# xmlyqing00/V-FloodNet

Hardware: AMD Instinct MI355X
Metric: segmented frames/sec at 480p (higher is better)
Workload: dtype f32

## Files before the change

### v-floodnet_amd/_lib.py

```python
import ctypes as C
import os
import re

import torch

_HERE = os.path.dirname(os.path.abspath(__file__))
LIB_PATH = os.environ.get('VFN_LIB_PATH') or os.path.join(_HERE, 'libvfn_hip.so')

_lib = None

c_fp = C.c_void_p

_SCALARS = {'int': C.c_int, 'float': C.c_float, 'double': C.c_double, 'long long': C.c_longlong}
_POINTEES = set(_SCALARS) | {'void', 'char', 'unsigned char', 'short', 'unsigned short', 'unsigned long long'}
_RENAMED = {'in': 'inp'}
_DECLARATOR = re.compile(r'(?:const\s+)?([A-Za-z_][\w ]*?)(?:\s*(\*)\s*|\s+)(\w+)\s*(?:\[([^\]]*)\])?')


def parse_header(text, known_structs=None):
    defines, enums, structs, protos = {}, {}, dict(known_structs or {}), {}

    def fail(why, decl):
        raise RuntimeError(f'vfn_hip.h: {why}: {" ".join(decl.split())[:120]!r}')

# ... 48 lines not shown
        depth += (ch == '{') - (ch == '}')
        if depth < 0:
            fail('unbalanced declaration', text[start:pos + 1])
        if ch == ';' and depth == 0:
            decls.append(text[start:pos])
            start = pos + 1
    if text[start:].strip():
        fail('unbalanced declaration', text[start:])

    for decl in decls:
        m = re.fullmatch(r'\s*enum\s*\{(.*)\}\s*', decl, flags=re.S)
        if m:
            value = -1
            for item in m.group(1).split(','):
                name, _, expr = item.partition('=')
                value = number(expr, decl) if expr.strip() else value + 1
                enums[name.strip()] = value
            continue
        m = re.fullmatch(r'\s*typedef\s+struct\s*(\w*)\s*\{(.*)\}\s*(\w+)\s*', decl, flags=re.S)
        if m:
            if m.group(1) not in ('', m.group(3)):
                fail('struct tag and typedef name differ', decl)
            fields = []
            for member in m.group(2).split(';'):
                if member.strip():
                    first, *more = member.split(',')
                    head = _DECLARATOR.fullmatch(first.strip())
                    if more and (not head or head.group(2)):
                        fail('several declarators after a pointer', member)
                    fields.append(declarator(first, member, False))
                    fields += [declarator(f'{head.group(1)} {item}', member, False) for item in more]
            structs[m.group(3)] = type(m.group(3), (C.Structure,), {'_fields_': fields})
            continue
        m = re.fullmatch(r'\s*int\s+(vfn_\w+)\s*\((.*)\)\s*', decl, flags=re.S)
        if m:
            if m.group(1) in protos:
                fail('declared twice', decl)
            params = m.group(2).strip()
            protos[m.group(1)] = [] if params == 'void' else [declarator(p, decl, True)[1] for p in params.split(',')]
            continue
        fail('declaration not understood', decl)
    return defines, enums, {k: v for k, v in structs.items() if k not in (known_structs or {})}, protos


with open(os.path.join(os.path.dirname(_HERE), 'include', 'vfn_hip.h')) as _f:
    DEFINES, ENUMS, STRUCTS, SIGNATURES = parse_header(_f.read())
ALL_SYMBOLS = sorted(SIGNATURES)
with open(os.path.join(os.path.dirname(_HERE), 'include', 'vfn_winograd6.h')) as _f:
    SIGNATURES_WINOGRAD6 = parse_header(_f.read())[3]
with open(os.path.join(os.path.dirname(_HERE), 'include', 'vfn_image_val.h')) as _f:
    DEFINES_IMAGE_VAL, _, _, SIGNATURES_IMAGE_VAL = parse_header(_f.read())
with open(os.path.join(os.path.dirname(_HERE), 'include', 'vfn_shortcut_fused.h')) as _f:
    SIGNATURES_SHORTCUT_FUSED = parse_header(_f.read(), STRUCTS)[3]
SEG_SCORES_CHUNK, SEG_SCORES_MAX_BLOCKS = DEFINES_IMAGE_VAL['VFN_SEG_SCORES_CHUNK'], DEFINES_IMAGE_VAL['VFN_SEG_SCORES_MAX_BLOCKS']
ABI_VERSION = DEFINES['VFN_ABI_VERSION']
TRAIN_AUG_MAX_T, TRAIN_AUG_MAX_SIDE, TRAIN_AUG_MAX_OUT, TRAIN_AUG_MAX_OBJ = (
    DEFINES['VFN_TRAIN_AUG_MAX_' + _k] for _k in ('T', 'SIDE', 'OUT', 'OBJ'))

ConvDesc = STRUCTS['vfn_conv_desc']
WgradDesc = STRUCTS['vfn_wgrad_desc']
RefreshFilter = STRUCTS['vfn_refresh_filter']
RefreshEpilogue = STRUCTS['vfn_refresh_epilogue']
GatherEntry = STRUCTS['vfn_gather_entry']
StemDesc = STRUCTS['vfn_stem_desc']
BankScanDesc = STRUCTS['vfn_bankscan_desc']
MemReadDesc = STRUCTS['vfn_memread_desc']
BankMatchDesc = STRUCTS['vfn_bankmatch_desc']
BankDesc = STRUCTS['vfn_bank_desc']
TrainAugFrame = STRUCTS['vfn_train_aug_frame']
TrainAugDesc = STRUCTS['vfn_train_aug_desc']

DESC_IDS = {ENUMS['VFN_DESC_' + _k]: _c for _k, _c in (
    ('CONV', ConvDesc), ('STEM', StemDesc), ('BANKSCAN', BankScanDesc), ('MEMREAD', MemReadDesc), ('BANK', BankDesc),
    ('WGRAD', WgradDesc), ('REFRESH_FILTER', RefreshFilter), ('REFRESH_EPILOGUE', RefreshEpilogue), ('GATHER', GatherEntry),
    ('BANKMATCH', BankMatchDesc), ('TRAIN_AUG', TrainAugDesc))}


def lib():
    global _lib
    if _lib is None:
        if not os.path.isfile(LIB_PATH):
            raise RuntimeError(
                f'{LIB_PATH} not found: build the HIP kernels first '
                '(python -c "import __graft_entry__ as g; g.build()" or make -C v-floodnet_amd/csrc)')
        L = C.CDLL(LIB_PATH)

        def declare(name, signatures=SIGNATURES, header='vfn_hip.h'):
            if not hasattr(L, name):
                raise RuntimeError(f'{LIB_PATH} lacks {name}, which include/{header} declares: rebuild it (make -C v-floodnet_amd/csrc)')
            fn = getattr(L, name)
            fn.argtypes, fn.restype = signatures[name], C.c_int
            return fn

        if declare('vfn_abi_version')() != ABI_VERSION:
            raise RuntimeError(f'{LIB_PATH} has ABI version {L.vfn_abi_version()}, this package expects {ABI_VERSION} '
                               '(descriptor layouts differ): rebuild it (make -C v-floodnet_amd/csrc)')
        declare('vfn_sizeof_desc')
        for which, cls in DESC_IDS.items():
            if L.vfn_sizeof_desc(which) != C.sizeof(cls):
                raise RuntimeError(f'{LIB_PATH}: sizeof({cls.__name__}) is {L.vfn_sizeof_desc(which)} in the library, '
                                   f'{C.sizeof(cls)} in this binding: rebuild it (make -C v-floodnet_amd/csrc)')
        for name in SIGNATURES:
            declare(name)
        for name in SIGNATURES_WINOGRAD6:
            declare(name, SIGNATURES_WINOGRAD6, 'vfn_winograd6.h')
        for name in SIGNATURES_IMAGE_VAL:
            declare(name, SIGNATURES_IMAGE_VAL, 'vfn_image_val.h')
        for name in SIGNATURES_SHORTCUT_FUSED:
            declare(name, SIGNATURES_SHORTCUT_FUSED, 'vfn_shortcut_fused.h')
        _lib = L
    return _lib


def check(status, what):
    if status != 0:
        raise RuntimeError(f'HIP kernel launcher {what} failed with status {status}')


def ptr(t):
    if t is None:
        return None
    return C.c_void_p(t.data_ptr())


_raw_stream = getattr(torch._C, '_cuda_getCurrentRawStream', None)


def stream():
    if _raw_stream is not None:
        return C.c_void_p(_raw_stream(torch.cuda.current_device()))
    return C.c_void_p(torch.cuda.current_stream().cuda_stream)


def require_gpu(t, what='tensor'):
    if not t.is_cuda:
        raise RuntimeError(f'{what} must live on the GPU: the V-FloodNet hot path has no CPU fallback')


PROBES = []


def independent_stream(device, beside=(), tries=12, priority=0):
    device = torch.device(device)
    cur = torch.cuda.current_stream(device)
    others = [cur] + [s_ for s_ in beside if s_ is not None]
    big, small = torch.zeros(16 * 1024 * 1024, device=device), torch.zeros(16, device=device)

    def overlaps(cand, ref):
        torch.cuda.synchronize(device)
        ref_end, cand_end = torch.cuda.Event(), torch.cuda.Event()
        with torch.cuda.stream(ref):
            for _ in range(64):
                big.add_(1.0)
            ref_end.record()
        with torch.cuda.stream(cand):
            small.add_(1.0)
            cand_end.record()
        cand_end.synchronize()
        ok = not ref_end.query()
        torch.cuda.synchronize(device)
        return ok

# ... 11 lines not shown
```

### v-floodnet_amd/engine.py

```python
import math
import os

import torch

from . import _lib, ops, weights as W
from ._lib import ptr, stream, check, MemReadDesc, BankScanDesc
from .feature_bank import pick_nsplit, pick_scan_slices, MAX_SPLIT, MAX_SPLIT_SCAN, QT_SCAN, DK, DV

_CFG_EFF = {(128, 128): 1.00, (128, 64): 0.95, (64, 128): 0.95, (64, 64): 0.86, (32, 64): 0.74,
            (64, 32): 0.74, (128, 32): 0.80, (256, 128): 0.97}
_CFG_TILES = None
_TUNED = {}
_TUNED_PATH = __import__('os').path.join(__import__('os').path.dirname(__import__('os').path.abspath(__file__)),
                                         'tuned_gfx950.json')
_TUNED_BF16 = {}
_TUNED_BF16_PATH = _TUNED_PATH.replace('tuned_gfx950.json', 'tuned_gfx950_bf16.json')
_TUNED_BF16X3 = {}
_TUNED_BF16X3_PATH = _TUNED_PATH.replace('tuned_gfx950.json', 'tuned_gfx950_bf16x3.json')
_TABLES = (_TUNED, _TUNED_BF16, _TUNED_BF16X3)
_TABLE_PATHS = (_TUNED_PATH, _TUNED_BF16_PATH, _TUNED_BF16X3_PATH)
_TUNED_WINO6 = {}
_TUNED_WINO6_PATH = _TUNED_PATH.replace('tuned_gfx950.json', 'tuned_gfx950_wino6.json')
_TUNED_SHORTCUT = {}
_TUNED_SHORTCUT_PATH = _TUNED_PATH.replace('tuned_gfx950.json', 'tuned_gfx950_shortcut.json')


def is_wino6_desc(d):
    return d.w_batch_rows > 0 and d.M == 64 * d.w_batch_rows


def table_of(d, mode):
    return _TUNED_WINO6 if mode == 0 and is_wino6_desc(d) else _TABLES[mode]


def _load_tuned():
    import json
    import os
    if os.environ.get('VFN_IGNORE_TUNED') == '1':
        return
    for path, table in zip(_TABLE_PATHS + (_TUNED_WINO6_PATH,), _TABLES + (_TUNED_WINO6,)):
        alt = os.environ.get('VFN_TUNED_DIR')
        if alt and os.path.isfile(os.path.join(alt, os.path.basename(path))):
            path = os.path.join(alt, os.path.basename(path))
        if os.path.isfile(path):
            for k, v in json.load(open(path)).items():
                t = (int(v[0]), int(v[1]), int(v[2]) if len(v) > 2 else 0)
                table[tuple(int(x) for x in k.split(','))] = t + tuple(int(x) for x in v[3:6]) if len(v) >= 6 else t
    path = _TUNED_SHORTCUT_PATH
    alt = os.environ.get('VFN_TUNED_DIR')
    if alt and os.path.isfile(os.path.join(alt, os.path.basename(path))):
        path = os.path.join(alt, os.path.basename(path))
    if os.path.isfile(path):
        for k, v in json.load(open(path)).items():
            _TUNED_SHORTCUT[tuple(int(x) for x in k.split(','))] = (int(v[0]), int(v[1]))


def save_tuned(path=None, mode=0):
    import json
    table = _TUNED_WINO6 if mode == 'wino6' else _TUNED_SHORTCUT if mode == 'shortcut' else _TABLES[mode]
    with open(path or (_TUNED_WINO6_PATH if mode == 'wino6' else _TUNED_SHORTCUT_PATH if mode == 'shortcut' else _TABLE_PATHS[mode]), 'w') as f:
        json.dump({','.join(str(x) for x in k): list(v) for k, v in sorted(table.items())}, f, indent=0)


_load_tuned()


def pad_divide_by(h, w, d=16):
    new_h = h + d - h % d if h % d > 0 else h
    new_w = w + d - w % d if w % d > 0 else w
    lh = int((new_h - h) / 2)
    uh = int(new_h - h) - lh
    lw = int((new_w - w) / 2)
    uw = int(new_w - w) - lw
    return (lw, uw, lh, uh), new_h, new_w


WS_FLOATS = 16 * 1024 * 1024
_WINOGRAD_TRAIN = os.environ.get('VFN_WINOGRAD_TRAIN', '1') == '1'
_BATCH_MEMREAD = os.environ.get('VFN_TRAIN_BATCH_MEMREAD', '1') == '1'
MAX_GROUP = 16
_TRAIN_SLOTS = int(os.environ.get('VFN_TRAIN_SLOTS', 2))
_WINOGRAD = os.environ.get('VFN_WINOGRAD', '1')
_WINOGRAD_F6 = os.environ.get('VFN_WINOGRAD_F6', '1')
_WINO_ROWS32 = os.environ.get('VFN_WINO_ROWS32', '1')
_SHORTCUT_FUSED = os.environ.get('VFN_SHORTCUT_FUSED', '1')
_WINOGRAD_LP = os.environ.get('VFN_WINOGRAD_LP', '1') == '1'
_WINOGRAD_MIN_M = int(os.environ.get('VFN_WINOGRAD_MIN_M', 10000))
_WINO_TABLE = {}
_WINO_TABLE_BF16 = {}
_WINO_PATH = os.path.join(os.path.dirname(os.path.abspath(__file__)), 'wino_gfx950.json')
if os.environ.get('VFN_IGNORE_TUNED') != '1':
    for _path, _tab in ((_WINO_PATH, _WINO_TABLE), (_WINO_PATH.replace('.json', '_bf16.json'), _WINO_TABLE_BF16)):
        if os.path.isfile(_path):
            _tab.update({tuple(int(x) for x in k.split(',')): int(v) for k, v in __import__('json').load(open(_path)).items()})
_INLAUNCH_SPLITK = __import__('os').environ.get('VFN_INLAUNCH_SPLITK', '1') == '1'


def _tiles():
    global _CFG_TILES
    if _CFG_TILES is None:
        _CFG_TILES = ops.conv_cfg_tiles()
    return _CFG_TILES


def apply_choice(desc, choice, ws, counters=None):
    cfg, ks, split_from = choice[:3]
    if ks > 1 and (desc.out_ld % 4 or (desc.res and desc.res_ld % 4)):
        ks, split_from = 1, 0
    if cfg >= ops.PCONV_CFG0 and not ops.pconv_eligible(desc, 0):
        fb = tuple(choice[3:6]) if len(choice) >= 6 else choose_cfg(desc.M, desc.Cout, desc.KH * desc.KW * desc.Cin, 0, use_table=False)
        return apply_choice(desc, fb, ws, counters)
    if cfg >= ops.WINO_GEMM_CFG0:
        ops.set_splitk(desc, 1, None)
        return cfg
    if ops.conv_cfg_kind(cfg) == 2:
        if counters is None or ws is None or ws.numel() < ops.SK_WS_FLOATS:
            ws, counters = ops.streamk_scratch(ws.device if ws is not None else torch.device('cuda', torch.cuda.current_device()))
        ops.set_streamk(desc, ws, counters)
        return cfg
    if ks > 1:
        bm, bn = _tiles()[cfg]
        n_tiles = (desc.Cout + bn - 1) // bn
        rows = desc.M - (split_from // n_tiles) * bm
        if desc.Cout % bn or not _INLAUNCH_SPLITK or ops.conv_cfg_kind(cfg) != 0 or desc.w_packed or desc.in_lp or desc.out_lp:
            counters = None
        ops.set_splitk(desc, ks, ws, split_from, rows, counters)
    else:
        ops.set_splitk(desc, 1, None)
    return cfg


def _scores_buffer(p, fb):
    if os.environ.get('VFN_STORE_SCORES', '1') == '0':
        return None
    per_obj = ((fb._cap + 63) // 64) * ((p.HW + 127) // 128) * 8192
    if fb.obj_n * per_obj * 4 > float(os.environ.get('VFN_SCORES_MAX_GB', 48)) * 2 ** 30:
        return None
    key = (fb.obj_n, per_obj)
# ... 379 lines not shown
    def all_lists(self):
        out = [self.mem]
        for qs in self.qsets:
            out += [qs.pre[1], qs.pre[2], qs.post[0], qs.post[1]]
        for qs in self._qbatch.values():
            out += [qs.pre[qs.nq]]
            if qs._dec_batch is not None:
                out += [qs._dec_batch.post]
        return out

    def batch_set(self, n):
        qs = self._qbatch.get(n)
        if qs is None:
            qs = self._qbatch[n] = QuerySet(self, nq=n)
            qs.build()
        return qs

    def _trunk_buffers(self, N):
        dev = self.eng.device
        f = lambda *s: torch.empty(*s, device=dev, dtype=torch.float32)
        b = {}
        b['r1'] = f(N, self.h2, self.w2, 64)
        b['x4'] = f(N, self.h4, self.w4, 64)
        for name, (h, w, planes) in {'res2': (self.h4, self.w4, 64), 'res3': (self.h8, self.w8, 128),
                                     'res4': (self.h16, self.w16, 256)}.items():
            hin, win = (h * 2, w * 2) if name != 'res2' else (h, w)
            b[name] = dict(t1a=f(N, hin, win, planes), t1=f(N, h, w, planes), t2=f(N, h, w, planes),
                           ds=f(N, h, w, planes * 4), o=[f(N, h, w, planes * 4) for _ in range(2)],
                           out=f(N, h, w, planes * 4))
        return b

    def _lp_args(self, out):
        if not self.eng.any_x3 or out.shape[-1] % 32:
            return ()
        self._lp_state[(out.data_ptr(), tuple(out.shape))] = True
        return (self.lp_twin(out), True)

    def lp_twin(self, t):
        st = t.untyped_storage()
        key = st.data_ptr()
        if key not in self._twins:
            self._twins[key] = torch.empty(st.nbytes() // 4, dtype=torch.float32, device=t.device)
        return torch.as_strided(self._twins[key], t.size(), t.stride(), t.storage_offset())

    def has_lp(self, t, relu):
        return self._lp_state.get((t.data_ptr(), tuple(t.shape))) == bool(relu)

    def _conv(self, lst, layer, x, out, N, H, Wd, res=None, relu_in=False, relu_out=False, name='conv',
              in_ld=None, out_ld=None, res_mod=0, lp_out=None, f32_out=True):
        bf = self.eng.layer_mode(name)
        lp = bf == 2
        if self.eng.mixed:
            f32_out = True
        if ((bf == 0 or (bf == 1 and _WINOGRAD_LP and not self.keep_acts and layer.cin % 64 == 0)) and in_ld is None and
                (_WINOGRAD_TRAIN or not self.keep_acts) and x.shape[-1] == layer.cin and self.eng.use_winograd(layer, N * H * Wd, bf)):
            tile = 6 if (bf == 0 and not self.keep_acts and res_mod % (H * Wd) == 0 and
                         self.eng.winograd_tile(layer, N * H * Wd) == 6) else 4
            return self._conv_winograd(lst, layer, x, out, N, H, Wd, res, relu_in, relu_out, name, out_ld, res_mod, bf, tile)
        d = ops.make_conv_desc(x, layer.w, layer.cout, layer.k, layer.k, layer.stride, layer.pad, out,
                               layer.scale, layer.shift, res, relu_in, relu_out,
                               cin=layer.cin, in_ld=in_ld if in_ld is not None else x.shape[-1],
                               out_ld=out_ld, N=N, H=H, W=Wd)
        d.res_mod = int(res_mod)
        if lp and in_ld is None and layer.cin % 32 == 0 and self.has_lp(x, relu_in):
            d.inp, d.in_lp, d.relu_in = ptr(self.lp_twin(x)), 1, 0
        if lp and lp_out and layer.cout % 32 == 0 and d.out_ld % 32 == 0:
            d.out_lp, d.out_lp_relu = ptr(self.lp_twin(out)), int(lp_out == 'relu')
            self._lp_state[(out.data_ptr(), tuple(out.shape))] = (lp_out == 'relu')
            if not f32_out:
                d.out = None
        else:
            self._lp_state.pop((out.data_ptr(), tuple(out.shape)), None)
        K = layer.k * layer.k * layer.cin
        if bf == 1 and layer.cin % 64:
            bf = 2
        if bf:
            ops.use_packed_weights(d, layer.w_lp(bf))
        choice = choose_cfg(d.M, layer.cout, K, bf)
        if choice[1] > 1 and (d.out_ld % 4 or (res is not None and d.res_ld % 4)):
            choice = (choice[0], 1, 0)
        cfg = apply_choice(d, choice, self._ws_cur, self._cnt_cur)
        lst.append(Launch(ops.conv2d_launch, (d, cfg, bf), f'{name}[{d.M}x{layer.cout}x{K}]', 2.0 * d.M * layer.cout * K))
        return out

    def _conv_winograd(self, lst, layer, x, out, N, H, Wd, res, relu_in, relu_out, name, out_ld, res_mod, bf=0, tile=4):
        comps = 64 if tile == 6 else 36
        rows = ops.winograd6_rows(N, H, Wd) if tile == 6 else ops.winograd_rows(N, H, Wd)
        if tile == 6 and bf == 0 and _WINO_ROWS32 != '0':
            rows32 = (ops.winograd6_tiles(N, H, Wd) + 31) // 32 * 32
            c32 = _TUNED_WINO6.get((64 * rows32, layer.cout, layer.cin))
            if rows32 < rows and (_WINO_ROWS32 == '2' or (c32 is not None and ops.is_wino_gemm32_cfg(c32[0]))):
                rows = rows32
        key = id(self._ws_cur)
        need_v, need_m = comps * rows * layer.cin, comps * rows * layer.cout
        V, Mb = self._wino.get(key, (None, None))
        if V is None or V.numel() < need_v or Mb.numel() < need_m:
            dev = self.eng.device
            V = torch.zeros(max(need_v, V.numel() if V is not None else 0), device=dev)
            Mb = torch.empty(max(need_m, Mb.numel() if Mb is not None else 0), device=dev)
            self._wino[key] = (V, Mb)
        Mb = Mb[:need_m].view(comps * rows, layer.cout)
        if bf == 1:
            V = V.view(torch.bfloat16)[:need_v].view(36 * rows, layer.cin)
            U = layer.w_wino_bf16()
        else:
            V = V[:need_v].view(comps * rows, layer.cin)
            U = layer.w_wino6() if tile == 6 else layer.w_wino()
        lst.append(Launch(ops.winograd_input, (x, V, rows, relu_in, N, H, Wd, layer.cin, x.shape[-1], tile), name + '.wino_in'))
        dg = ops.make_winograd_gemm_desc(V, U, Mb, rows, layer.cin, layer.cout, comps)
        if bf:
            choice = _TABLES[bf].get((dg.M, layer.cout, layer.cin))
            if choice is None or choice[0] < ops.WINO_GEMM_CFG0:
                tc = 5 if rows % 64 == 0 and layer.cout >= 128 and rows >= 1024 else 3
                choice = (ops.wino_gemm_cfg(tc, 512), 1, 0)
        elif tile == 6:
            choice = _TUNED_WINO6.get((dg.M, layer.cout, layer.cin))
            if choice is None or choice[0] not in ops.wino_gemm_cfg_options(rows, layer.cout):
                choice = ((ops.wino_gemm32_cfg(4 if layer.cout >= 128 else 5, 768) if rows % 64 else
                           ops.wino_gemm_cfg(5 if layer.cout >= 128 else 7, 768)), 1, 0)
        else:
            choice = choose_cfg(dg.M, layer.cout, layer.cin, 0)
        cfg = apply_choice(dg, choice, self._ws_cur, self._cnt_cur)
        lst.append(Launch(ops.conv2d_launch, (dg, cfg, bf), f'{name}.wino_gemm[{dg.M}x{layer.cout}x{layer.cin}]', 2.0 * dg.M * layer.cout * layer.cin))
        self._lp_state.pop((out.data_ptr(), tuple(out.shape)), None)
        lst.append(Launch(ops.winograd_output, (Mb, rows, out, N, H, Wd, layer.cout, layer.scale, layer.shift, res,
                                                res.shape[-1] if res is not None else 0, res_mod, relu_out,
                                                out_ld if out_ld is not None else out.shape[-1], tile), name + '.wino_out'))
        return out

    def _trunk(self, lst, enc, bufs, N, prefix, acts=None):
        x = bufs['x4']
        lst.append(Launch(ops.maxpool3x3s2, (bufs['r1'], x), prefix + '.maxpool'))
        H, Wd = self.h4, self.w4
        for lname in ('res2', 'res3', 'res4'):
            blocks = enc[lname]
            lb = bufs[lname]
            for bi, blk in enumerate(blocks):
                s = blk['conv2'].stride
                Ho, Wo = H // s, Wd // s
                t1 = lb['t1a'] if (s == 2) else lb['t1']
                t2, ds_buf = lb['t2'], lb['ds']
                if self.keep_acts:
                    t1, t2 = torch.empty_like(t1), torch.empty_like(lb['t2'])
                    ds_buf = torch.empty_like(lb['ds'])
                nm = f'{prefix}.{lname}.{bi}'
                self._conv(lst, blk['conv1'], x, t1, N, H, Wd, relu_out=True, name=nm + '.conv1', lp_out='plain', f32_out=False)
                self._conv(lst, blk['conv2'], t1, t2, N, H, Wd, relu_out=True, name=nm + '.conv2', lp_out='plain',
                           f32_out=False)
                out = lb['out'] if bi == len(blocks) - 1 else lb['o'][bi % 2]
                if self.keep_acts and bi != len(blocks) - 1:
                    out = torch.empty_like(out)
                if 'down' in blk and self._shortcut_fused(lst, blk, x, t2, out, N, H, Wd, Ho, Wo, nm):
                    idn = None
                elif 'down' in blk:
                    self._conv(lst, blk['down'], x, ds_buf, N, H, Wd, name=nm + '.down')
                    idn = ds_buf
                else:
                    idn = x
                if idn is not None:
                    self._conv(lst, blk['conv3'], t2, out, N, Ho, Wo, res=idn, relu_out=True, name=nm + '.conv3',
                               lp_out='plain')
# ... 709 lines not shown
        m.q = ptr(kv_q)
        m.qv = None
        m.bank_k, m.bank_v, m.bank_len, m.ml, m.o_part = ptr(fb._kbuf), ptr(fb._vbuf), ptr(fb._len_dev), ptr(p.ml), ptr(p.o_part)
        m.cnt = ptr(fb._cnt) if update_bank else None
        m.info, m.out = ptr(fb._ibuf), ptr(out)
        m.stride_k, m.stride_v, m.stride_cnt, m.stride_info = cap * DK, cap * DV, cap, cap * 2
        m.scale, m.thres = scale, 1e-3
        m.ldq, m.ldqv, m.ld_out, m.HW, m.obj_n = DK + DV, DK + DV, out.shape[-1], HW, K
        m.precision = mr_mode
        m.nsplit = pick_nsplit(HW, K, fb.len_upper(), QT_SCAN, MAX_SPLIT)
        if klp is not None:
            m.bank_k_lp, m.bank_v_lp = ptr(klp), ptr(vlp)
        if scores is not None:
            m.scores, m.stride_scores = ptr(scores), scores.shape[1]
        check(L.vfn_memread_apply(_lib.C.byref(m), s), 'vfn_memread_apply')
        check(L.vfn_memread_finish(_lib.C.byref(m), s), 'vfn_memread_finish')

    def capture(self, H0, W0, obj_n, group=0):
        p = self.plan(H0, W0, obj_n)
        if not _GRAPHS or self.eager or p.keep_acts:
            return 0
        before = p.graphs.captures
        torch.cuda.current_stream().synchronize()
        p.graphs.warm(p.mem)
        for qs in p.qsets:
            for n in qs.sizes:
                lst = qs.pre[n]
                p.graphs.warm(lst)
                if 0 < qs.split[n] < len(lst):
                    p.graphs.warm(lst, 0, qs.split[n])
                    p.graphs.warm(lst, qs.split[n], None)
            for L in qs.post:
                p.graphs.warm(L)
        for G in ([group] if group and group > 1 else []):
            qs = p.batch_set(G)
            b = qs.dec_batch()
            if self.refresher._tables is None:
                self._settle()
            p.graphs.warm(qs.pre[G])
            p.graphs.warm(b.post)
        torch.cuda.current_stream().synchronize()
        return p.graphs.captures - before

    def autotune(self, H0, W0, obj_n, iters=3, only_missing=False, shape_filter=None, cfg_filter=None):
        p = self.plan(H0, W0, obj_n)
        seen = {}
        side_sets = list(p.qsets) + ([] if p.keep_acts else list(p._qbatch.values()))
        side_lists = [id(qs.pre[n]) for qs in side_sets for n in qs.sizes]
        for lst in p.all_lists():
            for l in lst:
                l_side = id(lst) in side_lists
                if l.fn is ops.conv2d_launch:
                    d = l.args[0]
                    key = (d.M, d.Cout, d.KH * d.KW * d.Cin, int(l.args[2]), is_wino6_desc(d))
                    if only_missing and key[:3] in table_of(d, key[3]):
                        continue
                    if shape_filter is not None and not shape_filter(key[:3]):
                        continue
                    seen.setdefault(key, []).append((l, l_side))
        for key, launches in seen.items():
            d = launches[0][0].args[0]
            bf = key[3]
            if key[4]:
                best = tune_desc(d, bf, p.ws, p.cnt, iters=iters, cfg_filter=lambda k_, c_: c_ >= ops.WINO_GEMM_CFG0 and (cfg_filter is None or cfg_filter(k_, c_)))
            else:
                best = tune_desc(d, bf, p.ws, p.cnt, iters=iters, cfg_filter=cfg_filter)
            table_of(d, bf)[key[:3]] = best
            for l, in_q in launches:
                l.args = (l.args[0], apply_choice(l.args[0], best, p.ws_q if in_q else p.ws, p.cnt_q if in_q else p.cnt), bf)
        if seen:
            p.graphs.invalidate()
        return dict(_TABLES[self.mode])
```

### v-floodnet_amd/ops.py

```python
import ctypes as C
import os

import torch

from . import _lib
from ._lib import ptr, stream, check, ConvDesc


_cfg_tiles = None


def conv_cfg_tiles():
    global _cfg_tiles
    if _cfg_tiles is None:
        L = _lib.lib()
        out = []
        for c in range(L.vfn_conv_cfg_count()):
            bm, bn = C.c_int(), C.c_int()
            L.vfn_conv_cfg_tile(c, C.byref(bm), C.byref(bn))
            out.append((bm.value, bn.value))
        _cfg_tiles = tuple(out)
    return _cfg_tiles


# ... 208 lines not shown


def pconv_cfg(tile_cfg, wgs=512):
    return PCONV_CFG0 + int(tile_cfg) + 8 * (int(wgs) // 128)


def pconv_eligible(desc, mode=0):
    lim = 0x7fffff00
    return (mode == 0 and desc.KH == 1 and desc.KW == 1 and desc.stride == 1 and desc.pad == 0 and not desc.mask and not desc.in_lp and
            not desc.out_lp and not desc.w_packed and not desc.w_batch_rows and desc.Cin % 32 == 0 and desc.in_ld % 4 == 0 and
            desc.M >= 1 and desc.M == desc.N * desc.H * desc.W and desc.M * desc.in_ld * 4 < lim and desc.M * desc.out_ld * 4 < lim and
            desc.cout_pad * desc.Cin * 4 < lim and
            (not desc.res or (desc.res_mod if desc.res_mod > 0 else desc.M) * desc.res_ld * 4 < lim))


def shortcut_fused_eligible(sc, main, mode=0):
    lim = 0x7fffff00
    for d in (sc, main):
        if (d.KH != 1 or d.KW != 1 or d.pad != 0 or d.mask or d.in_lp or d.out_lp or d.w_packed or d.ksplit > 1 or d.w_batch_rows or d.res or
                d.Cin < 32 or d.Cin % 32 or d.in_ld < d.Cin or d.in_ld % 4 or d.N < 1 or d.H < 1 or d.W < 1 or not d.inp or not d.w):
            return False
    return (mode == 0 and bool(main.out) and main.stride == 1 and sc.stride in (1, 2) and main.M >= 1 and main.M == main.N * main.H * main.W and
            sc.Ho == (sc.H - 1) // sc.stride + 1 and sc.Wo == (sc.W - 1) // sc.stride + 1 and sc.M == sc.N * sc.Ho * sc.Wo and
            sc.M == main.M and sc.Cout == main.Cout and main.Cout >= 1 and main.out_ld >= main.Cout and
            min(sc.cout_pad, main.cout_pad) >= (main.Cout + 63) // 64 * 64 and
            sc.N * sc.H * sc.W * sc.in_ld * 4 < lim and main.M * main.in_ld * 4 < lim and main.M * main.out_ld * 4 < lim and
            main.cout_pad * main.Cin * 4 < lim and sc.cout_pad * sc.Cin * 4 < lim)


def shortcut_fused_cfg_options(sc, main):
    out = []
    for tc in range(4):
        bn = WINO_GEMM_TILES[tc & 3][1]
        if (bn > 64 and main.Cout < 128) or min(sc.cout_pad, main.cout_pad) < (main.Cout + bn - 1) // bn * bn:
            continue
        out += [(tc, w) for w in (256, 512, 768)]
    return out


def shortcut_fused_launch(sc, main, tile_cfg, wgs):
    check(_lib.lib().vfn_conv1x1_shortcut_fused_f32(C.byref(sc), C.byref(main), int(tile_cfg), int(wgs), stream()),
          'vfn_conv1x1_shortcut_fused_f32')


def pconv_cfg_options(cout):
    out = []
    for tc in range(8):
        if WINO_GEMM_TILES[tc & 3][1] > 64 and cout < 128:
            continue
        out += [pconv_cfg(tc, w) for w in (256, 512, 768)]
    return out


def conv2d_launch(desc, cfg, mode=0):
    cfg = int(cfg)
    if cfg >= PCONV_CFG0:
        c = cfg - PCONV_CFG0
        if mode != 0:
            raise RuntimeError('the persistent 1x1 convolution is an f32 kernel')
        check(_lib.lib().vfn_conv1x1_persistent_f32(C.byref(desc), c & 7, (c >> 3) * 128, stream()), 'vfn_conv1x1_persistent_f32')
        return
    if cfg >= WINO_GEMM_CFG0:
        c, rows = cfg - WINO_GEMM_CFG0, desc.w_batch_rows
        if is_wino_gemm32_cfg(cfg):
            c = cfg - WINO_GEMM32_CFG0
            if mode != 0 or rows <= 0:
                raise RuntimeError('the 32-row tiles take an f32 Winograd-domain descriptor (w_batch_rows)')
            check(_lib.lib().vfn_winograd_gemm_f32(desc.inp, desc.w, desc.out, desc.M // rows, rows, desc.Cin, desc.Cout, desc.cout_pad,
                                                   8 + (c & 7), (c >> 3) * 128, stream()), 'vfn_winograd_gemm_f32')
            return
        if mode == 1 and rows > 0:
            check(_lib.lib().vfn_winograd_gemm_bf16(desc.inp, desc.w, desc.out, desc.M // rows, rows, desc.Cin, desc.Cout, desc.cout_pad, c & 7,
                                                    (c >> 3) * 128, stream()), 'vfn_winograd_gemm_bf16')
            return
        if mode != 0 or rows <= 0:
            raise RuntimeError('the persistent GEMM takes an f32 (or plain-bf16) Winograd-domain descriptor (w_batch_rows)')
        check(_lib.lib().vfn_winograd_gemm_f32(desc.inp, desc.w, desc.out, desc.M // rows, rows, desc.Cin, desc.Cout, desc.cout_pad, c & 7,
                                               (c >> 3) * 128, stream()), 'vfn_winograd_gemm_f32')
        return
    name = _CONV_FN[int(mode)]
    check(getattr(_lib.lib(), name)(C.byref(desc), cfg, stream()), name)


def conv_cfg_name(cfg, mode=0, _cache={}):
    cfg = int(cfg)
    if cfg >= WINO_GEMM_CFG0:
        bm, bn, wm, wn, pd, _ = persistent_cfg_info(cfg)
        return f'wino_gemm_kernel<{bm}, {bn}, {wm}, {wn}, {pd}, {"true" if cfg >= PCONV_CFG0 else "false"}, {"true" if mode == 1 else "false"}>'
    if mode not in _cache:
        _cache[mode] = conv_cfg_names(mode)
    return _cache[mode][cfg]


def conv2d_nhwc(x, wp, cout, kh, kw, stride, pad, scale=None, shift=None, res=None,
                relu_in=False, relu_out=False, cfg=3, out=None, mode=0):
    N, H, W, _ = x.shape
    Ho = (H + 2 * pad - kh) // stride + 1
    Wo = (W + 2 * pad - kw) // stride + 1
    if out is None:
        out = torch.empty(N, Ho, Wo, cout, device=x.device, dtype=torch.float32)
    d = make_conv_desc(x, wp, cout, kh, kw, stride, pad, out, scale, shift, res, relu_in, relu_out)
    if mode == 0 and conv_cfg_kind(cfg) == 2:
        set_streamk(d, *streamk_scratch(x.device))
    conv2d_launch(d, cfg, mode)
    return out


_WINO_G = torch.tensor([[1 / 4, 0, 0], [-1 / 6, -1 / 6, -1 / 6], [-1 / 6, 1 / 6, -1 / 6], [1 / 24, 1 / 12, 1 / 6], [1 / 24, -1 / 12, 1 / 6], [0, 0, 1]],
                       dtype=torch.float64)
WINO_ROW_MULT = 256
_WINO_KROT = int(os.environ.get('VFN_KROT', '0'))


def pack_winograd_weight(w):
    cout, cin = w.shape[0], w.shape[1]
    assert tuple(w.shape[2:]) == (3, 3)
    g = w.detach().double().cpu()
    U = torch.einsum('ia,ocab,jb->ijoc', _WINO_G, g, _WINO_G)
    cp = (cout + 255) // 256 * 256
    out = torch.zeros(36, cp, cin, dtype=torch.float32)
    out[:, :cout] = U.reshape(36, cout, cin).float()
    return out.reshape(36 * cp, cin).contiguous()


def winograd_rows(N, H, W):
    t = N * ((H + 3) // 4) * ((W + 3) // 4)
    return (t + WINO_ROW_MULT - 1) // WINO_ROW_MULT * WINO_ROW_MULT


_WINO6_G = torch.tensor([[1, 0, 0], [-2 / 9, -2 / 9, -2 / 9], [-2 / 9, 2 / 9, -2 / 9], [1 / 90, 1 / 45, 2 / 45], [1 / 90, -1 / 45, 2 / 45],
                         [32 / 45, 16 / 45, 8 / 45], [32 / 45, -16 / 45, 8 / 45], [0, 0, 1]], dtype=torch.float64)
WINO6_ROW_MULT = 64


def pack_winograd6_weight(w):
    cout, cin = w.shape[0], w.shape[1]
    assert tuple(w.shape[2:]) == (3, 3)
    g, G = w.detach().double().cpu(), _WINO6_G
# ... 15 lines not shown


def pack_winograd_weight_bf16(w):
    return pack_winograd_weight(w).to(torch.bfloat16).contiguous()


def winograd_input(x, V, rows_pad, relu, N=None, H=None, W=None, cin=None, ld_x=None, tile=4):
    if N is None:
        N, H, W = x.shape[0], x.shape[1], x.shape[2]
    cin = cin if cin is not None else x.shape[-1]
    ld_x = ld_x if ld_x is not None else x.shape[-1]
    if tile == 6:
        check(_lib.lib().vfn_winograd6_input_f32(ptr(x), N, H, W, cin, ld_x, int(relu), ptr(V), rows_pad, stream()), 'vfn_winograd6_input_f32')
        return
    if V.dtype == torch.bfloat16:
        check(_lib.lib().vfn_winograd_input_bf16(ptr(x), N, H, W, cin, ld_x, int(relu), ptr(V), rows_pad, stream()), 'vfn_winograd_input_bf16')
        return
    check(_lib.lib().vfn_winograd_input_f32(ptr(x), N, H, W, cin, ld_x, int(relu), ptr(V), rows_pad, stream()), 'vfn_winograd_input_f32')


def winograd_output(Mb, rows_pad, out, N, H, W, cout, scale, shift, res, res_ld, res_mod, relu_out, out_ld=None, tile=4):
    name = 'vfn_winograd6_output_f32' if tile == 6 else 'vfn_winograd_output_f32'
    check(getattr(_lib.lib(), name)(ptr(Mb), rows_pad, N, H, W, cout, ptr(scale), ptr(shift), ptr(res), int(res_ld), int(res_mod),
                                    int(relu_out), ptr(out), out_ld if out_ld is not None else out.shape[-1], stream()), name)


def make_winograd_gemm_desc(V, U, Mb, rows_pad, cin, cout, comps=36):
    d = make_conv_desc(V, U, cout, 1, 1, 1, 0, Mb, None, None, None, False, False, cin=cin, in_ld=cin, out_ld=cout, N=1, H=1, W=comps * rows_pad)
    d.cout_pad = U.shape[0] // comps
    d.w_batch_rows = rows_pad
    d.k_rot = _WINO_KROT
    return d


def winograd_gemm(V, U, Mb, rows_pad, cin, cout, cfg=0, wgs=0, comps=36):
    check(_lib.lib().vfn_winograd_gemm_f32(ptr(V), ptr(U), ptr(Mb), comps, rows_pad, cin, cout, U.shape[0] // comps, int(cfg), int(wgs), stream()),
          'vfn_winograd_gemm_f32')


def conv2d_winograd(x, w, scale=None, shift=None, res=None, relu_in=False, relu_out=False, cfg=2, res_mod=0, tile=4):
    N, H, W, cin = x.shape
    cout = w.shape[0]
    if tile == 6:
        comps, rows, tiles = 64, winograd6_rows(N, H, W), winograd6_tiles(N, H, W)
        U = pack_winograd6_weight(w).to(x.device)
    else:
        comps, rows, tiles = 36, winograd_rows(N, H, W), vfn_winograd_tiles(N, H, W)
        U = pack_winograd_weight(w).to(x.device)
    V = torch.empty(comps * rows, cin, device=x.device, dtype=torch.float32)
    Mb = torch.empty(comps * rows, cout, device=x.device, dtype=torch.float32)
    out = torch.empty(N, H, W, cout, device=x.device, dtype=torch.float32)
    if rows > tiles and tile != 6:
        V.view(comps, rows, cin)[:, tiles:].zero_()
    winograd_input(x, V, rows, relu_in, tile=tile)
    d = make_winograd_gemm_desc(V, U, Mb, rows, cin, cout, comps)
    if conv_cfg_kind(cfg) == 2:
        set_streamk(d, *streamk_scratch(x.device))
    conv2d_launch(d, cfg, 0)
    winograd_output(Mb, rows, out, N, H, W, cout, scale, shift, res, res.shape[-1] if res is not None else 0, res_mod, relu_out, tile=tile)
    return out


def vfn_winograd_tiles(N, H, W):
    return N * ((H + 3) // 4) * ((W + 3) // 4)


def make_stem_desc(frame, mask, w, scale, shift, out, mean, std, N, H0, W0, pad, Hp, Wp):
    from ._lib import StemDesc
    d = StemDesc()
    d.frame, d.mask, d.w, d.scale, d.shift, d.out = ptr(frame), ptr(mask), ptr(w), ptr(scale), ptr(shift), ptr(out)
    for i in range(3):
        d.mean[i] = float(mean[i])
        d.std[i] = float(std[i])
    d.N, d.cin = N, (5 if mask is not None else 3)
    d.H0, d.W0 = H0, W0
    d.pad_top, d.pad_left = pad[2], pad[0]
    d.Hp, d.Wp, d.Ho, d.Wo = Hp, Wp, Hp // 2, Wp // 2
    return d


def stem_launch(desc):
    check(_lib.lib().vfn_stem_conv7x7_f32(C.byref(desc), stream()), 'vfn_stem_conv7x7_f32')


def pack_stem_weight(ws):
    w = torch.cat([x.detach().float() for x in ws], dim=1)
    P = w.shape[1]
    out = torch.zeros(P, 7, 8, 64, dtype=torch.float32, device=w.device)
    out[:, :, :7, :] = w.permute(1, 2, 3, 0)
    return out.reshape(P * 56, 64).contiguous()


def maxpool3x3s2(x, out):
    N, H, W, Cc = x.shape
    check(_lib.lib().vfn_maxpool3x3s2_nhwc_f32(ptr(x), ptr(out), N, H, W, Cc, stream()), 'vfn_maxpool3x3s2_nhwc_f32')
    return out


def upsample2x_add(s, pm, out, s_bcast, out_lp=None, lp_relu=False):
    N, h, w, Cc = out.shape
    if out_lp is not None:
        check(_lib.lib().vfn_upsample2x_add_lp_nhwc_f32(ptr(s), ptr(pm), ptr(out), ptr(out_lp), int(lp_relu), N, h, w, Cc,
                                                        int(s_bcast), stream()), 'vfn_upsample2x_add_lp_nhwc_f32')
        return out
    check(_lib.lib().vfn_upsample2x_add_nhwc_f32(ptr(s), ptr(pm), ptr(out), N, h, w, Cc, int(s_bcast), stream()),
          'vfn_upsample2x_add_nhwc_f32')
    return out
# ... 458 lines not shown
```

Before: 167.8.

## Add LDS-resident thin 3x3 conv kernel and strided-input Winograd F6 path

Adds a persistent HIP kernel for 3x3 stride-1 convolutions with 32 output channels and 32 or 64 input channels. It keeps the whole filter bank and an input patch tile in LDS, uses f32 MFMA, and prefetches the next tile's patch plus the residual values while computing, with an XCD-aware tile split. Layers are routed to this kernel only when the tuned thin table has an entry for them. The change also lets Winograd F6 take inputs with a strided leading dimension instead of falling back to direct conv. The risk is that the thin path stays inactive without a tuned JSON file, and correctness hinges on the new kernel's boundary handling.

```diff
diff --git a/include/vfn_conv_thin.h b/include/vfn_conv_thin.h
--- /dev/null
+++ b/include/vfn_conv_thin.h
@@ -0,0 +1,16 @@
+#ifndef VFN_CONV_THIN_H
+#define VFN_CONV_THIN_H
+
+#define VFN_THIN3X3_MAX_WGS 2048
+
+#ifdef __cplusplus
+extern "C" {
+#endif
+
+int vfn_conv3x3_thin_f32(const vfn_conv_desc* d, int cfg, void* stream);
+
+#ifdef __cplusplus
+}
+#endif
+
+#endif
diff --git a/v-floodnet_amd/_lib.py b/v-floodnet_amd/_lib.py
--- a/v-floodnet_amd/_lib.py
+++ b/v-floodnet_amd/_lib.py
@@ -124,6 +124,8 @@
     DEFINES_IMAGE_VAL, _, _, SIGNATURES_IMAGE_VAL = parse_header(_f.read())
 with open(os.path.join(os.path.dirname(_HERE), 'include', 'vfn_shortcut_fused.h')) as _f:
     SIGNATURES_SHORTCUT_FUSED = parse_header(_f.read(), STRUCTS)[3]
+with open(os.path.join(os.path.dirname(_HERE), 'include', 'vfn_conv_thin.h')) as _f:
+    DEFINES_CONV_THIN, _, _, SIGNATURES_CONV_THIN = parse_header(_f.read(), STRUCTS)
 SEG_SCORES_CHUNK, SEG_SCORES_MAX_BLOCKS = DEFINES_IMAGE_VAL['VFN_SEG_SCORES_CHUNK'], DEFINES_IMAGE_VAL['VFN_SEG_SCORES_MAX_BLOCKS']
 ABI_VERSION = DEFINES['VFN_ABI_VERSION']
 TRAIN_AUG_MAX_T, TRAIN_AUG_MAX_SIDE, TRAIN_AUG_MAX_OUT, TRAIN_AUG_MAX_OBJ = (
@@ -180,6 +182,8 @@
             declare(name, SIGNATURES_IMAGE_VAL, 'vfn_image_val.h')
         for name in SIGNATURES_SHORTCUT_FUSED:
             declare(name, SIGNATURES_SHORTCUT_FUSED, 'vfn_shortcut_fused.h')
+        for name in SIGNATURES_CONV_THIN:
+            declare(name, SIGNATURES_CONV_THIN, 'vfn_conv_thin.h')
         _lib = L
     return _lib
 
diff --git a/v-floodnet_amd/csrc/conv_thin3x3.hip b/v-floodnet_amd/csrc/conv_thin3x3.hip
--- /dev/null
+++ b/v-floodnet_amd/csrc/conv_thin3x3.hip
@@ -0,0 +1,201 @@
+#include "common.h"
+#include "conv_internal.h"
+#include "../../include/vfn_conv_thin.h"
+
+template <int CIN>
+struct thin_geom {
+    static constexpr int TH = 8, TW = 16;
+    static constexpr int PH = TH + 2, PW = TW + 2;
+    static constexpr int S = CIN + 4;
+    static constexpr int RP = (PW * S + 63) / 64 * 64;
+    static constexpr int CH = CIN / 4;
+    static constexpr int NCH = PH * PW * CH;
+    static constexpr int PC = (NCH + 255) / 256;
+    static constexpr int W_FLOATS = 9 * 32 * S;
+    static constexpr int P_FLOATS = PH * RP;
+    static constexpr size_t LDS_BYTES = (size_t)(W_FLOATS + P_FLOATS) * sizeof(float);
+};
+
+template <int CIN>
+__global__ __launch_bounds__(256)
+void conv_thin3x3_kernel(const vfn_conv_desc p, int tiles_x, int tiles_y, int total, int res_imgs) {
+    using G = thin_geom<CIN>;
+    constexpr int S = G::S, RP = G::RP, CH = G::CH, PC = G::PC;
+    extern __shared__ __attribute__((aligned(16))) char smem[];
+    float* sW = reinterpret_cast<float*>(smem);
+    float* sP = sW + G::W_FLOATS;
+
+    const int tid = threadIdx.x, lane = tid & 63, wave = tid >> 6;
+    const int li = lane & 31, lh = lane >> 5;
+
+    int first, step, n_my;
+    if ((gridDim.x & 7) == 0) {
+        const int gx = (int)gridDim.x >> 3, xcd = (int)blockIdx.x & 7, loc = (int)blockIdx.x >> 3;
+        const int q = total >> 3, r8 = total & 7;
+        const int u_begin = xcd < r8 ? xcd * (q + 1) : r8 * (q + 1) + (xcd - r8) * q;
+        const int u_end = u_begin + q + (xcd < r8 ? 1 : 0);
+        first = u_begin + loc;
+        step = gx;
+        n_my = first < u_end ? (u_end - first + gx - 1) / gx : 0;
+    } else {
+        first = blockIdx.x;
+        step = gridDim.x;
+        n_my = first < total ? (total - first + step - 1) / step : 0;
+    }
+    if (n_my == 0) return;
+
+    constexpr int OOB = 0x7ffffff0;
+    const __amdgpu_buffer_rsrc_t rs_in = __builtin_amdgcn_make_buffer_rsrc(
+        const_cast<float*>(p.in), 0, (int)((size_t)p.N * p.H * p.W * p.in_ld * sizeof(float)), 0x00020000);
+    const int res_rows = res_imgs > 0 ? res_imgs * p.H * p.W : p.M;
+    const __amdgpu_buffer_rsrc_t rs_res = __builtin_amdgcn_make_buffer_rsrc(
+        const_cast<float*>(p.res), 0, p.res ? (int)((size_t)res_rows * p.res_ld * sizeof(float)) : 0, 0x00020000);
+
+    int c_py[PC], c_px[PC], c_lds[PC], c_off[PC];
+#pragma unroll
+    for (int j = 0; j < PC; ++j) {
+        const int q = tid + j * 256;
+        const int pix = q / CH, ch = q - pix * CH;
+        const int py = pix / G::PW, px = pix - py * G::PW;
+        c_py[j] = q < G::NCH ? py : (1 << 29);
+        c_px[j] = px;
+        c_lds[j] = py * RP + px * S + ch * 4;
+        c_off[j] = ((py * p.W + px) * p.in_ld + ch * 4) * (int)sizeof(float);
+    }
+    struct blk { int n, y0, x0; };
+    auto block_of = [&](int t) {
+        const int tx = t % tiles_x, tyn = t / tiles_x;
+        return blk{tyn / tiles_y, (tyn % tiles_y) * G::TH, tx * G::TW};
+    };
+    auto load_chunk = [&](const blk& b, bool live, int j, f32x4& r) {
+        const int base = (((b.n * p.H + b.y0 - 1) * p.W + b.x0 - 1) * p.in_ld) * (int)sizeof(float);
+        const bool ok = live && (unsigned)(b.y0 - 1 + c_py[j]) < (unsigned)p.H && (unsigned)(b.x0 - 1 + c_px[j]) < (unsigned)p.W;
+        r = __builtin_bit_cast(f32x4, __builtin_amdgcn_raw_buffer_load_b128(rs_in, ok ? base + c_off[j] : OOB, 0, 0));
+    };
+    const float relu_floor = p.relu_in ? 0.f : -INFINITY;
+    auto store_patch = [&](const f32x4 (&r)[PC]) {
+#pragma unroll
+        for (int j = 0; j < PC; ++j) {
+            if ((j + 1) * 256 <= G::NCH || tid + j * 256 < G::NCH) {
+                f32x4 v = r[j];
+#pragma unroll
+                for (int e = 0; e < 4; ++e) v[e] = vfn_floor_nan(v[e], relu_floor);
+                *reinterpret_cast<f32x4*>(sP + c_lds[j]) = v;
+            }
+        }
+    };
+
+    f32x4 pre[PC];
+    {
+        const blk b0 = block_of(first);
+#pragma unroll
+        for (int j = 0; j < PC; ++j) load_chunk(b0, true, j, pre[j]);
+    }
+
+    {
+        constexpr int WC = 32 * 9 * CH / 256;
+        static_assert(WC * 256 == 32 * 9 * CH, "the filter bank is a whole number of chunks per thread");
+        f32x4 wv[WC];
+#pragma unroll
+        for (int j = 0; j < WC; ++j) wv[j] = *reinterpret_cast<const f32x4*>(p.w + (size_t)(tid + j * 256) * 4);
+#pragma unroll
+        for (int j = 0; j < WC; ++j) {
+            const int q = tid + j * 256;
+            const int f = q / (9 * CH), k4 = q - f * (9 * CH);
+            const int tap = k4 / CH, ch = k4 - tap * CH;
+            *reinterpret_cast<f32x4*>(sW + (tap * 32 + f) * S + ch * 4) = wv[j];
+        }
+    }
+
+    const float sc = p.scale ? p.scale[li] : 1.f;
+    const float sh = p.shift ? p.shift[li] : 0.f;
+    const float* aBase = sP + (2 * wave + (li >> 4)) * RP + (li & 15) * S + 4 * lh;
+    const float* bBase = sW + li * S + 4 * lh;
+    constexpr int KB = CIN / 8, STEPS = 9 * KB;
+    constexpr int PSTEP = (STEPS - 1 - 16) / PC;
+    static_assert(PSTEP >= 1, "more patch chunks than steps left");
+
+    for (int i = 0; i < n_my; ++i) {
+        const int t = first + i * step;
+        store_patch(pre);
+        __syncthreads();
+        const bool has_next = i + 1 < n_my;
+        const blk b = block_of(t), bn = block_of(has_next ? t + step : t);
+        const int y_w = b.y0 + 2 * wave, x_l = b.x0 + 4 * lh;
+        const int nr = res_imgs > 0 ? b.n % res_imgs : b.n;
+        const int res_pix = (nr * p.H + y_w) * p.W + x_l, out_pix = (b.n * p.H + y_w) * p.W + x_l;
+        float rv[16];
+
+        f32x16 acc;
+#pragma unroll
+        for (int r = 0; r < 16; ++r) acc[r] = 0.f;
+        auto read_frags = [&](int s, f32x4& a, f32x4& bf) {
+            const int tap = s / KB, kb = s - tap * KB;
+            const int kh = tap / 3, kw = tap - kh * 3;
+            a = *reinterpret_cast<const f32x4*>(aBase + kh * RP + kw * S + kb * 8);
+            bf = *reinterpret_cast<const f32x4*>(bBase + tap * 32 * S + kb * 8);
+        };
+        f32x4 fa[2], fb[2];
+        read_frags(0, fa[0], fb[0]);
+#pragma unroll
+        for (int s = 0; s < STEPS; ++s) {
+            if (s + 1 < STEPS) read_frags(s + 1, fa[(s + 1) & 1], fb[(s + 1) & 1]);
+            if (s < 16) {
+                const int dy = s >> 3, dx = (s & 3) + 8 * ((s >> 2) & 1);
+                const bool ok = y_w + dy < p.H && x_l + dx < p.W;
+                rv[s] = __builtin_bit_cast(float, __builtin_amdgcn_raw_buffer_load_b32(
+                    rs_res, ok ? ((res_pix + dy * p.W + dx) * p.res_ld + li) * (int)sizeof(float) : OOB, 0, 0));
+            } else if ((s - 16) % PSTEP == 0 && (s - 16) / PSTEP < PC) {
+                load_chunk(bn, has_next, (s - 16) / PSTEP, pre[(s - 16) / PSTEP]);
+            }
+            __builtin_amdgcn_sched_barrier(0);
+#pragma unroll
+            for (int e = 0; e < 4; ++e)
+                acc = __builtin_amdgcn_mfma_f32_32x32x2f32(fa[s & 1][e], fb[s & 1][e], acc, 0, 0, 0);
+            __builtin_amdgcn_sched_barrier(0);
+        }
+
+#pragma unroll
+        for (int r = 0; r < 16; ++r) {
+            const int dy = r >> 3, dx = (r & 3) + 8 * ((r >> 2) & 1);
+            if (y_w + dy < p.H && x_l + dx < p.W) {
+                float v = acc[r] * sc + sh;
+                if (p.res) v += rv[r];
+                if (p.relu_out) v = fmaxf(v, 0.f);
+                p.out[(size_t)(out_pix + dy * p.W + dx) * p.out_ld + li] = v;
+            }
+        }
+        __syncthreads();
+    }
+}
+
+template <int CIN>
+static int launch_thin(const vfn_conv_desc& d, int wgs, hipStream_t s) {
+    using G = thin_geom<CIN>;
+    static const bool lds_ok = vfn_allow_lds(conv_thin3x3_kernel<CIN>, G::LDS_BYTES);
+    (void)lds_ok;
+    const int tiles_x = (d.W + G::TW - 1) / G::TW, tiles_y = (d.H + G::TH - 1) / G::TH;
+    const long long total = (long long)d.N * tiles_y * tiles_x;
+    if (total >= 0x7fffff00LL) return VFN_ERR_ARG;
+    int grid = wgs > 0 ? wgs : 256;
+    if (grid > total) grid = (int)total;
+    if (grid >= 8) grid &= ~7;
+    const int res_imgs = (d.res && d.res_mod > 0) ? d.res_mod / (d.H * d.W) : 0;
+    hipLaunchKernelGGL(conv_thin3x3_kernel<CIN>, dim3(grid), dim3(256), G::LDS_BYTES, s, d, tiles_x, tiles_y, (int)total, res_imgs);
+    return vfn_check_launch();
+}
+
+extern "C" int vfn_conv3x3_thin_f32(const vfn_conv_desc* d, int cfg, void* stream) {
+    if (!d || !d->in || !d->w || !d->out || cfg < 0 || cfg > VFN_THIN3X3_MAX_WGS) return VFN_ERR_ARG;
+    if (d->KH != 3 || d->KW != 3 || d->stride != 1 || d->pad != 1 || d->Cout != 32 || d->cout_pad < 32 || (d->Cin != 32 && d->Cin != 64))
+        return VFN_ERR_ARG;
+    if (d->N < 1 || d->H < 1 || d->W < 1 || d->Ho != d->H || d->Wo != d->W || d->M != d->N * d->H * d->W) return VFN_ERR_ARG;
+    if (d->in_ld < d->Cin || d->in_ld % 4 || d->out_ld < 32) return VFN_ERR_ARG;
+    if (d->mask || d->in_lp || d->out_lp || d->w_packed || d->w_batch_rows || d->ksplit > 1) return VFN_ERR_ARG;
+    const long long hw = (long long)d->H * d->W, lim = 0x7fffff00LL;
+    if (d->res && (d->res_ld < 32 || d->res_mod < 0 || (d->res_mod > 0 && d->res_mod % hw))) return VFN_ERR_ARG;
+    if ((long long)d->M * d->in_ld * 4 >= lim || (long long)d->M * d->out_ld * 4 >= lim ||
+        (d->res && (d->res_mod > 0 ? d->res_mod : (long long)d->M) * d->res_ld * 4 >= lim)) return VFN_ERR_ARG;
+    if ((reinterpret_cast<uintptr_t>(d->in) | reinterpret_cast<uintptr_t>(d->w)) & 15) return VFN_ERR_ARG;
+    return d->Cin == 64 ? launch_thin<64>(*d, cfg, (hipStream_t)stream) : launch_thin<32>(*d, cfg, (hipStream_t)stream);
+}
diff --git a/v-floodnet_amd/engine.py b/v-floodnet_amd/engine.py
--- a/v-floodnet_amd/engine.py
+++ b/v-floodnet_amd/engine.py
@@ -23,6 +23,8 @@
 _TUNED_WINO6_PATH = _TUNED_PATH.replace('tuned_gfx950.json', 'tuned_gfx950_wino6.json')
 _TUNED_SHORTCUT = {}
 _TUNED_SHORTCUT_PATH = _TUNED_PATH.replace('tuned_gfx950.json', 'tuned_gfx950_shortcut.json')
+_TUNED_THIN = {}
+_TUNED_THIN_PATH = _TUNED_PATH.replace('tuned_gfx950.json', 'tuned_gfx950_thin.json')
 
 
 def is_wino6_desc(d):
@@ -53,10 +55,20 @@
     if os.path.isfile(path):
         for k, v in json.load(open(path)).items():
             _TUNED_SHORTCUT[tuple(int(x) for x in k.split(','))] = (int(v[0]), int(v[1]))
+    path = _TUNED_THIN_PATH
+    if alt and os.path.isfile(os.path.join(alt, os.path.basename(path))):
+        path = os.path.join(alt, os.path.basename(path))
+    if os.path.isfile(path):
+        for k, v in json.load(open(path)).items():
+            _TUNED_THIN[tuple(int(x) for x in k.split(','))] = int(v)
 
 
 def save_tuned(path=None, mode=0):
     import json
+    if mode == 'thin':
+        with open(path or _TUNED_THIN_PATH, 'w') as f:
+            json.dump({','.join(str(x) for x in k): int(v) for k, v in sorted(_TUNED_THIN.items())}, f, indent=0)
+        return
     table = _TUNED_WINO6 if mode == 'wino6' else _TUNED_SHORTCUT if mode == 'shortcut' else _TABLES[mode]
     with open(path or (_TUNED_WINO6_PATH if mode == 'wino6' else _TUNED_SHORTCUT_PATH if mode == 'shortcut' else _TABLE_PATHS[mode]), 'w') as f:
         json.dump({','.join(str(x) for x in k): list(v) for k, v in sorted(table.items())}, f, indent=0)
@@ -84,6 +96,8 @@
 _WINOGRAD_F6 = os.environ.get('VFN_WINOGRAD_F6', '1')
 _WINO_ROWS32 = os.environ.get('VFN_WINO_ROWS32', '1')
 _SHORTCUT_FUSED = os.environ.get('VFN_SHORTCUT_FUSED', '1')
+_WINO_STRIDED_IN = os.environ.get('VFN_WINO_STRIDED_IN', '1')
+_THIN3X3 = os.environ.get('VFN_THIN3X3', '1')
 _WINOGRAD_LP = os.environ.get('VFN_WINOGRAD_LP', '1') == '1'
 _WINOGRAD_MIN_M = int(os.environ.get('VFN_WINOGRAD_MIN_M', 10000))
 _WINO_TABLE = {}
@@ -569,11 +583,12 @@
         lp = bf == 2
         if self.eng.mixed:
             f32_out = True
-        if ((bf == 0 or (bf == 1 and _WINOGRAD_LP and not self.keep_acts and layer.cin % 64 == 0)) and in_ld is None and
+        if ((bf == 0 or (bf == 1 and _WINOGRAD_LP and not self.keep_acts and layer.cin % 64 == 0)) and
                 (_WINOGRAD_TRAIN or not self.keep_acts) and x.shape[-1] == layer.cin and self.eng.use_winograd(layer, N * H * Wd, bf)):
             tile = 6 if (bf == 0 and not self.keep_acts and res_mod % (H * Wd) == 0 and
                          self.eng.winograd_tile(layer, N * H * Wd) == 6) else 4
-            return self._conv_winograd(lst, layer, x, out, N, H, Wd, res, relu_in, relu_out, name, out_ld, res_mod, bf, tile)
+            if in_ld is None or (tile == 6 and _WINO_STRIDED_IN != '0' and in_ld % 4 == 0 and in_ld >= layer.cin):
+                return self._conv_winograd(lst, layer, x, out, N, H, Wd, res, relu_in, relu_out, name, out_ld, res_mod, bf, tile, in_ld)
         d = ops.make_conv_desc(x, layer.w, layer.cout, layer.k, layer.k, layer.stride, layer.pad, out,
                                layer.scale, layer.shift, res, relu_in, relu_out,
                                cin=layer.cin, in_ld=in_ld if in_ld is not None else x.shape[-1],
@@ -589,6 +604,12 @@
         else:
             self._lp_state.pop((out.data_ptr(), tuple(out.shape)), None)
         K = layer.k * layer.k * layer.cin
+        thin = _TUNED_THIN.get((d.M, layer.cout, K)) if (bf == 0 and not self.keep_acts and _THIN3X3 != '0') else None
+        if (thin is not None and ops.is_thin3x3_cfg(thin) and ops.thin3x3_cfg_info(thin)[0] == layer.cin and d.res_mod % (H * Wd) == 0 and
+                ops.thin3x3_eligible(d, 0)):
+            ops.set_splitk(d, 1, None)
+            lst.append(Launch(ops.conv2d_launch, (d, thin, 0), f'{name}[{d.M}x{layer.cout}x{K}]', 2.0 * d.M * layer.cout * K))
+            return out
         if bf == 1 and layer.cin % 64:
             bf = 2
         if bf:
@@ -600,7 +621,7 @@
         lst.append(Launch(ops.conv2d_launch, (d, cfg, bf), f'{name}[{d.M}x{layer.cout}x{K}]', 2.0 * d.M * layer.cout * K))
         return out
 
-    def _conv_winograd(self, lst, layer, x, out, N, H, Wd, res, relu_in, relu_out, name, out_ld, res_mod, bf=0, tile=4):
+    def _conv_winograd(self, lst, layer, x, out, N, H, Wd, res, relu_in, relu_out, name, out_ld, res_mod, bf=0, tile=4, in_ld=None):
         comps = 64 if tile == 6 else 36
         rows = ops.winograd6_rows(N, H, Wd) if tile == 6 else ops.winograd_rows(N, H, Wd)
         if tile == 6 and bf == 0 and _WINO_ROWS32 != '0':
@@ -623,7 +644,8 @@
         else:
             V = V[:need_v].view(comps * rows, layer.cin)
             U = layer.w_wino6() if tile == 6 else layer.w_wino()
-        lst.append(Launch(ops.winograd_input, (x, V, rows, relu_in, N, H, Wd, layer.cin, x.shape[-1], tile), name + '.wino_in'))
+        lst.append(Launch(ops.winograd_input, (x, V, rows, relu_in, N, H, Wd, layer.cin, in_ld if in_ld is not None else x.shape[-1], tile),
+                          name + '.wino_in'))
         dg = ops.make_winograd_gemm_desc(V, U, Mb, rows, layer.cin, layer.cout, comps)
         if bf:
             choice = _TABLES[bf].get((dg.M, layer.cout, layer.cin))
@@ -1439,6 +1461,8 @@
                 l_side = id(lst) in side_lists
                 if l.fn is ops.conv2d_launch:
                     d = l.args[0]
+                    if ops.is_thin3x3_cfg(l.args[1]):
+                        continue
                     key = (d.M, d.Cout, d.KH * d.KW * d.Cin, int(l.args[2]), is_wino6_desc(d))
                     if only_missing and key[:3] in table_of(d, key[3]):
                         continue
diff --git a/v-floodnet_amd/ops.py b/v-floodnet_amd/ops.py
--- a/v-floodnet_amd/ops.py
+++ b/v-floodnet_amd/ops.py
@@ -284,8 +284,50 @@
     return out
 
 
+THIN3X3_CFG0 = 3000
+THIN3X3_MAX_WGS = _lib.DEFINES_CONV_THIN['VFN_THIN3X3_MAX_WGS']
+
+
+def thin3x3_cfg(cin, wgs=256):
+    assert cin in (32, 64) and 0 <= int(wgs) <= THIN3X3_MAX_WGS < 4096
+    return THIN3X3_CFG0 + 4096 * (cin == 32) + int(wgs)
+
+
+def is_thin3x3_cfg(cfg):
+    return THIN3X3_CFG0 <= int(cfg) < THIN3X3_CFG0 + 2 * 4096
+
+
+def thin3x3_cfg_info(cfg):
+    c = int(cfg) - THIN3X3_CFG0
+    return (32 if c >= 4096 else 64), c & 4095
+
+
+def thin3x3_eligible(desc, mode=0, ignore_split=False):
+    lim, hw = 0x7fffff00, desc.H * desc.W
+    return (mode == 0 and bool(desc.inp) and bool(desc.w) and bool(desc.out) and desc.KH == 3 and desc.KW == 3 and desc.stride == 1 and
+            desc.pad == 1 and desc.Cout == 32 and desc.cout_pad >= 32 and desc.Cin in (32, 64) and desc.N >= 1 and desc.H >= 1 and
+            desc.W >= 1 and desc.Ho == desc.H and desc.Wo == desc.W and desc.M == desc.N * hw and desc.in_ld >= desc.Cin and
+            desc.in_ld % 4 == 0 and desc.out_ld >= 32 and not desc.mask and not desc.in_lp and not desc.out_lp and not desc.w_packed and
+            not desc.w_batch_rows and (desc.ksplit <= 1 or ignore_split) and
+            (not desc.res or (desc.res_ld >= 32 and desc.res_mod >= 0 and desc.res_mod % hw == 0 and
+                              (desc.res_mod if desc.res_mod > 0 else desc.M) * desc.res_ld * 4 < lim)) and
+            desc.M * desc.in_ld * 4 < lim and desc.M * desc.out_ld * 4 < lim and (desc.inp | desc.w) % 16 == 0)
+
+
+def thin3x3_cfg_options(desc):
+    return [thin3x3_cfg(desc.Cin, w) for w in ((256, 512) if desc.Cin == 32 else (256,))]
+
+
 def conv2d_launch(desc, cfg, mode=0):
     cfg = int(cfg)
+    if is_thin3x3_cfg(cfg):
+        if mode != 0:
+            raise RuntimeError('the LDS-resident 3x3 convolution is an f32 kernel')
+        cin, wgs = thin3x3_cfg_info(cfg)
+        if cin != desc.Cin and desc.Cin in (32, 64):
+            raise RuntimeError(f'configuration {cfg} names the Cin = {cin} instantiation, the layer has Cin = {desc.Cin}')
+        check(_lib.lib().vfn_conv3x3_thin_f32(C.byref(desc), wgs, stream()), 'vfn_conv3x3_thin_f32')
+        return
     if cfg >= PCONV_CFG0:
         c = cfg - PCONV_CFG0
         if mode != 0:
@@ -316,6 +358,8 @@
 
 def conv_cfg_name(cfg, mode=0, _cache={}):
     cfg = int(cfg)
+    if is_thin3x3_cfg(cfg):
+        return f'conv_thin3x3_kernel<{thin3x3_cfg_info(cfg)[0]}>'
     if cfg >= WINO_GEMM_CFG0:
         bm, bn, wm, wn, pd, _ = persistent_cfg_info(cfg)
         return f'wino_gemm_kernel<{bm}, {bn}, {wm}, {wn}, {pd}, {"true" if cfg >= PCONV_CFG0 else "false"}, {"true" if mode == 1 else "false"}>'
@@ -437,7 +481,8 @@
     out = torch.empty(N, H, W, cout, device=x.device, dtype=torch.float32)
     if rows > tiles and tile != 6:
         V.view(comps, rows, cin)[:, tiles:].zero_()
-    winograd_input(x, V, rows, relu_in, tile=tile)
+    assert x.stride(3) == 1 and x.stride(1) == W * x.stride(2) and x.stride(0) == H * x.stride(1)
+    winograd_input(x, V, rows, relu_in, ld_x=x.stride(2), tile=tile)
     d = make_winograd_gemm_desc(V, U, Mb, rows, cin, cout, comps)
     if conv_cfg_kind(cfg) == 2:
         set_streamk(d, *streamk_scratch(x.device))
```

After: 169.5, median of 6. +1.0%, better.
